# hongfz16/AvatarCLIP

Measured on AMD Instinct MI355X. Metric: rays_per_sec_512x512_64spp_clip_guided_train_iter, higher is better.
Workload: dtype f16 (forward) / bf16 (gradient sweeps) MFMA operands, fp32 accumulate

## Files before the change

### avatarclip_amd/build.py

```python
import os
import subprocess
import sys
from concurrent.futures import ThreadPoolExecutor

HERE = os.path.dirname(os.path.abspath(__file__))
CSRC = os.path.join(HERE, "csrc")
LIB = os.path.join(HERE, os.environ.get("AVC_LIB_NAME", "libavc.so"))
SOURCES = ["avc_core.hip", "avc_mlp_fwd.hip", "avc_mlp_bwd.hip", "avc_wgrad.hip", "avc_rays.hip", "avc_vit.hip", "avc_vit_attn.hip", "avc_vit_gemm.hip", "avc_mcubes.hip", "avc_raster.hip", "avc_raster_grad.hip", "avc_raster_tex.hip", "avc_params.hip", "avc_glue.hip", "avc_drive.hip", "avc_rig.hip", "avc_preview.hip", "avc_smpl.hip", "avc_smpl_grad.hip", "avc_codebook.hip", "avc_bake.hip", "avc_preview_clip.hip"]
ABI_HEADER = os.path.join("..", "..", "include", "avc.h")
TEXTURE_HEADER = "avc_texture.h"
CODEBOOK_HEADER = "avc_codebook.h"
PREVIEW_CLIP_HEADER = "avc_preview_clip.h"
BAKE_HEADER = "avc_bake.h"
HEADERS = ["avc_common.h", "avc_stage.h", "avc_mlp.h", "avc_bwd_body.h", "avc_offsets_gen.h", "avc_raster.h", "avc_raster_grad.h", "avc_smpl.h", "avc_vit.h", ABI_HEADER,
           TEXTURE_HEADER, CODEBOOK_HEADER, BAKE_HEADER, "avc_preview.h", PREVIEW_CLIP_HEADER]
FLAGS = ["--offload-arch=gfx950", "-O3", "-std=c++17", "-fPIC", "-Wno-comment"]


def _hipcc():
    for c in (os.environ.get("HIPCC"), "/opt/rocm/bin/hipcc", "hipcc"):
        if c and (os.path.isabs(c) and os.path.exists(c) or not os.path.isabs(c)):
            return c
    return "hipcc"


def _stale(target, deps):
    if not os.path.exists(target):
        return True
    t = os.path.getmtime(target)
    return any(os.path.getmtime(d) > t for d in deps if os.path.exists(d))


def _gen_offsets():
    import importlib.util
    spec = importlib.util.spec_from_file_location("gen_offsets", os.path.join(os.path.dirname(HERE), "scripts", "gen_offsets.py"))
    mod = importlib.util.module_from_spec(spec)
    spec.loader.exec_module(mod)
# ... 35 lines not shown
```

### avatarclip_amd/csrc/avc_wgrad.hip

```cpp
#include "avc_common.h"
#include "../../include/avc.h"
#include <type_traits>

#define WG_TB_MAX 9
#define WG_TILES_MAX 18
#define WG_BUF_BYTES (WG_TILES_MAX * 2048)
constexpr int WG_DEPTH = 4;
constexpr int WG_DMA_AUX = 2;

struct WgRegions { const char* base[2]; long stride[2]; };

typedef short vs4 __attribute__((__vector_size__(4 * sizeof(short))));
typedef __attribute__((address_space(3))) char lds_char;

__device__ __forceinline__ void wait_vmcnt(int n) {
#define WG_W(k) case k: asm volatile("s_waitcnt vmcnt(" #k ")" ::: "memory"); break;
  switch (n) {
    WG_W(0) WG_W(1) WG_W(2) WG_W(3) WG_W(4) WG_W(5) WG_W(6) WG_W(7) WG_W(8) WG_W(9) WG_W(10) WG_W(11) WG_W(12) WG_W(13) WG_W(14) WG_W(15)
    WG_W(16) WG_W(17) WG_W(18) WG_W(19) WG_W(20) WG_W(21) WG_W(22) WG_W(23) WG_W(24) WG_W(25) WG_W(26) WG_W(27) WG_W(28) WG_W(29) WG_W(30)
    WG_W(31) WG_W(32) WG_W(33) WG_W(34) WG_W(35) WG_W(36)
    default: asm volatile("s_waitcnt vmcnt(0)" ::: "memory"); break;
  }
#undef WG_W
}
// ... 111 lines not shown
    if (ta >= ta_n) continue;
#pragma unroll
    for (int k = 0; k < NK; ++k) {
      const int tb = wb + WB * k;
      if (tb >= tb_n) continue;
      f4* d4 = reinterpret_cast<f4*>(dst + ((long)(ta * tb_n + tb) * 64 + lane) * 16);
#pragma unroll
      for (int q = 0; q < 4; ++q) {
        f4 v;
        v[0] = acc[i * NK + k][4 * q]; v[1] = acc[i * NK + k][4 * q + 1]; v[2] = acc[i * NK + k][4 * q + 2]; v[3] = acc[i * NK + k][4 * q + 3];
        d4[q] = v;
      }
    }
    if (bias_partial && wb == i) {
      const float s = xhalf_sum(bsum[i]);
      if (lane < 32) bias_partial[(long)split * bias_elems + ta * 32 + lane] = s;
    }
  }
}

template <int N>
__device__ __forceinline__ void wait_vmcnt_imm() { asm volatile("s_waitcnt vmcnt(%0)" ::"n"(N) : "memory"); }

template <int MC, int TA, int TYA, int TYB>
struct WgCopies {
  const char* next[MC];
  long step[MC];
  unsigned src_lo;
  int wv;
  __device__ __forceinline__ WgCopies(const WgRegions& rg, int pa, int pb, long b0, int wv_, int lane) : wv(wv_) {
    src_lo = (((lane >> 2) & 3) * 32 + 4 * (lane >> 4) + (lane & 3)) * 16;
#pragma unroll
    for (int j = 0; j < MC; ++j) {
      const int c = wv + 8 * j, tix = c >> 1;
      const bool in_a = tix < TA;
      step[j] = in_a ? rg.stride[TYA] : rg.stride[TYB];
      next[j] = (in_a ? rg.base[TYA] + (long)(pa + tix) * 2048 : rg.base[TYB] + (long)(pb + tix - TA) * 2048) + b0 * step[j] + (c & 1) * 256;
    }
  }
  __device__ __forceinline__ void issue(char* lds, int slot) {
#pragma unroll
    for (int j = 0; j < MC; ++j) {
      asm("" : "+s"(next[j]));
      __builtin_amdgcn_global_load_lds((const __attribute__((address_space(1))) void*)(next[j] + src_lo),
                                       (__attribute__((address_space(3))) void*)(lds + slot * WG_BUF_BYTES + (wv + 8 * j) * 1024), 16, 0,
                                       WG_DMA_AUX);
      next[j] += step[j];
    }
  }
};

template <int MC, class Copies, class Contract>
__device__ __forceinline__ void wg_ring(char* lds, Copies& cp, long b0, long b1, Contract&& contract) {
  constexpr int depth = WG_DEPTH;
  const int n = (int)(b1 - b0);
  for (int d = 0; d < depth - 1; ++d)
    if (d < n) cp.issue(lds, d);
  int slot = 0;
  auto block = [&](auto ahead) {
    asm volatile("s_waitcnt lgkmcnt(0)" ::: "memory");
    __builtin_amdgcn_s_barrier();
    __builtin_amdgcn_sched_barrier(0);
    if constexpr (decltype(ahead)::value) cp.issue(lds, slot == 0 ? depth - 1 : slot - 1);
    contract(lds + slot * WG_BUF_BYTES);
    if (++slot == depth) slot = 0;
// ... 9 lines not shown
    wait_vmcnt(younger * MC);
    block(std::false_type{});
  }
}

__device__ __forceinline__ int wg_lane_off(int lane) {
  return (((lane >> 5) * 2) * 16 + (((lane >> 4) & 1) * 2 + (lane & 1)) * 4 + ((lane & 15) >> 2)) * 16 + 8 * ((lane & 3) >> 1);
}
__device__ __forceinline__ void wg_store_tile(float* dst, int tile, int lane, const facc& v16) {
  f4* d4 = reinterpret_cast<f4*>(dst + ((long)tile * 64 + lane) * 16);
#pragma unroll
  for (int q = 0; q < 4; ++q) {
    f4 v;
    v[0] = v16[4 * q]; v[1] = v16[4 * q + 1]; v[2] = v16[4 * q + 2]; v[3] = v16[4 * q + 3];
    d4[q] = v;
  }
}
__device__ __forceinline__ float wg_row_sum(float bsum, b8 s0, b8 s1) {
#pragma unroll
  for (int j = 0; j < 8; ++j) bsum += (float)s0[j] + (float)s1[j];
  return bsum;
}

template <int NI, int NK, int TA, int TB, int WA, int TYA, int TYB, bool BIAS, bool LASTA, bool LASTB, bool HI>
__device__ __forceinline__ void weight_grad_fixed(char* lds, const WgRegions& rg, int pa, int pb, long nblk, float* __restrict__ partial,
                                                  float* __restrict__ bias_partial, int out_elems, int bias_elems) {
  constexpr int WB = 8 / WA, nchunk = 2 * (TA + TB);
  constexpr int MC = HI ? (nchunk + 7) / 8 : nchunk / 8;
  constexpr int NIW = LASTA ? NI : NI - 1, NKW = LASTB ? NK : NK - 1;
  static_assert(WA * (NI - 1) < TA && WA * (NI - 2) + WA - 1 < TA && WB * (NK - 1) < TB && WB * (NK - 2) + WB - 1 < TB,
                "only the last slot of either side may be missing for some waves");
  const int lane = threadIdx.x & 63;
  const int wv = __builtin_amdgcn_readfirstlane((int)(threadIdx.x >> 6)) & 7;
  const int wa = wv % WA, wb = wv / WA;
  const int split = blockIdx.x, nsplit = gridDim.x;
  const long b0 = nblk * split / nsplit, b1 = nblk * (split + 1) / nsplit;
  WgCopies<MC, TA, TYA, TYB> cp(rg, pa, pb, b0, wv, lane);
  const int lane_off = wg_lane_off(lane);
  facc acc[NI * NK];
#pragma unroll
  for (int q = 0; q < NI * NK; ++q)
#pragma unroll
    for (int r = 0; r < 16; ++r) acc[q][r] = 0.f;
  float bsum = 0.f;
  wg_ring<MC>(lds, cp, b0, b1, [&](char* slot_buf) {
    lds_char* buf = (lds_char*)slot_buf + lane_off;
    b8 a[NI][2], bv[NK][2];
    auto read = [&](int t) {
#pragma unroll
      for (int i = 0; i < NIW; ++i) a[i][t] = tr_frag(buf + (wa + WA * i) * 2048, t);
#pragma unroll
      for (int k = 0; k < NKW; ++k) bv[k][t] = tr_frag(buf + (TA + wb + WB * k) * 2048, t);
    };
    auto convert = [&](int t) {
      if constexpr (TYA == 0) {
#pragma unroll
        for (int i = 0; i < NIW; ++i) a[i][t] = f16_to_bf16(a[i][t]);
      }
      if constexpr (TYB == 0) {
#pragma unroll
        for (int k = 0; k < NKW; ++k) bv[k][t] = f16_to_bf16(bv[k][t]);
      }
    };
    auto mfmas = [&](int t) {
#pragma unroll
      for (int i = 0; i < NIW; ++i)
#pragma unroll
        for (int k = 0; k < NKW; ++k) acc[i * NK + k] = MF<b8>::mma(a[i][t], bv[k][t], acc[i * NK + k]);
    };
    read(0);
    __builtin_amdgcn_sched_barrier(0);
    convert(0);
    __builtin_amdgcn_sched_barrier(0);
    read(1);
    mfmas(0);
    __builtin_amdgcn_sched_barrier(0);
    convert(1);
    mfmas(1);
    if constexpr (BIAS) {
      b8 s0 = a[0][0], s1 = a[0][1];
#pragma unroll
      for (int i = 1; i < NIW; ++i) { s0 = wb == i ? a[i][0] : s0; s1 = wb == i ? a[i][1] : s1; }
      bsum = wg_row_sum(bsum, s0, s1);
    }
  });
  float* dst = partial + (long)split * out_elems;
#pragma unroll
  for (int i = 0; i < NIW; ++i)
#pragma unroll
    for (int k = 0; k < NKW; ++k) wg_store_tile(dst, (wa + WA * i) * TB + wb + WB * k, lane, acc[i * NK + k]);
  if constexpr (BIAS) {
    if (wb < NIW) {
      const float s = xhalf_sum(bsum);
      if (lane < 32) bias_partial[(long)split * bias_elems + (wa + WA * wb) * 32 + lane] = s;
    }
  }
}

template <int NI, int NK, int TA, int TB, int WA, int TYA, int TYB, bool BIAS>
__device__ __forceinline__ void weight_grad_shipped(char* lds, const WgRegions& rg, int pa, int pb, long nblk, float* __restrict__ partial,
                                                    float* __restrict__ bias_partial, int out_elems, int bias_elems) {
  constexpr int WB = 8 / WA, nchunk = 2 * (TA + TB);
  constexpr bool role_a = WA * (NI - 1) + WA - 1 >= TA, role_b = WB * (NK - 1) + WB - 1 >= TB, role_hi = (nchunk & 7) != 0;
  const int wv = __builtin_amdgcn_readfirstlane((int)(threadIdx.x >> 6)) & 7;
  const bool lasta = !role_a || wv % WA + WA * (NI - 1) < TA, lastb = !role_b || wv / WA + WB * (NK - 1) < TB;
  const bool hi = !role_hi || wv < (nchunk & 7);
#define WG_ROLE(LA, LB, H)                                                                                                            \
  if ((LA || role_a) && (LB || role_b) && (H || role_hi) && lasta == LA && lastb == LB && hi == H)                                  \
    return weight_grad_fixed<NI, NK, TA, TB, WA, TYA, TYB, BIAS, LA || !role_a, LB || !role_b, H || !role_hi>(                        \
        lds, rg, pa, pb, nblk, partial, bias_partial, out_elems, bias_elems);
  WG_ROLE(true, true, true) WG_ROLE(true, true, false) WG_ROLE(true, false, true) WG_ROLE(true, false, false)
  WG_ROLE(false, true, true) WG_ROLE(false, true, false) WG_ROLE(false, false, true) WG_ROLE(false, false, false)
#undef WG_ROLE
}

template <int ROLE, int TYA, int TYB, bool BIAS>
__device__ __forceinline__ void weight_grad_fixed_9x9(char* lds, const WgRegions& rg, int pa, int pb, long nblk, float* __restrict__ partial,
                                                      float* __restrict__ bias_partial, int out_elems, int bias_elems) {
  constexpr int TA = 9, TB = 9;
  constexpr bool COL1 = ROLE >= 2, HAS_X = ROLE != 1;
  constexpr int MC = COL1 ? 4 : 5;
  constexpr int NR = COL1 ? 4 : 5;
  constexpr int XK = COL1 ? 0 : 4;
  const int lane = threadIdx.x & 63;
  const int wv = __builtin_amdgcn_readfirstlane((int)(threadIdx.x >> 6)) & 7;
  const int wa = wv & 3;
  const int split = blockIdx.x, nsplit = gridDim.x;
  const long b0 = nblk * split / nsplit, b1 = nblk * (split + 1) / nsplit;
  WgCopies<MC, TA, TYA, TYB> cp(rg, pa, pb, b0, wv, lane);
  const int lane_off = wg_lane_off(lane);
  int tb_of[NR];
#pragma unroll
  for (int k = 0; k < NR; ++k) tb_of[k] = COL1 ? 1 + 2 * ((wa + k) & 3) : 2 * k;
  facc acc[2 * NR], ex[2];
#pragma unroll
  for (int q = 0; q < 2 * NR; ++q)
// ... 198 lines not shown
      store_tile(wa, wb + 2 * k, acc[k]);
      store_tile(wa + 4, wb + 2 * k, acc[5 + k]);
    }
  }
  if (has_x) store_tile(8, wb + 2 * xk, ex[0]);
  if (wb == 1) store_tile(8, 2 * wa, ex[1]);
  if (bias_partial) {
#pragma unroll
    for (int i = 0; i < 2; ++i) {
      if (wb == i) {
        const float sx = xhalf_sum(bsum[i]);
        if (lane < 32) bias_partial[(long)split * bias_elems + (wa + 4 * i) * 32 + lane] = sx;
      }
    }
    if (wv == 4) {
      const float sx = xhalf_sum(xsum);
      if (lane < 32) bias_partial[(long)split * bias_elems + 8 * 32 + lane] = sx;
    }
  }
}

#define WG_MAX_PAIRS 24
struct WgPairs { int v[WG_MAX_PAIRS][8]; };
__global__ __launch_bounds__(512) void weight_grad_all_kernel(WgRegions rg, WgPairs pp, long nblk,
                                                              float* __restrict__ partial, float* __restrict__ bias_partial,
                                                              int out_elems, int bias_elems) {
  extern __shared__ __attribute__((aligned(16))) char lds[];
  const int* d = pp.v[blockIdx.y];
  float* bp = d[5] >= 0 ? bias_partial + d[5] : nullptr;
#define WG_ARGS lds, rg, d[0], d[1], d[2], d[3], d[6], d[7], nblk, partial + d[4], bp, out_elems, bias_elems
#define WG_SHIPPED(...) weight_grad_shipped<__VA_ARGS__>(lds, rg, d[0], d[2], nblk, partial + d[4], bp, out_elems, bias_elems)
  const bool gxf_bias = d[6] == 1 && d[7] == 0 && bp, fxg_plain = d[6] == 0 && d[7] == 1 && !bp;
  if (gxf_bias && d[1] == 8 && d[3] == 8) {
    WG_SHIPPED(4, 2, 8, 8, 2, 1, 0, true);
  } else if (fxg_plain && d[1] == 8 && d[3] == 8) {
    WG_SHIPPED(2, 4, 8, 8, 4, 0, 1, false);
  } else if (gxf_bias && d[1] == 7 && d[3] == 8) {
    WG_SHIPPED(4, 2, 7, 8, 2, 1, 0, true);
  } else if (fxg_plain && d[1] == 7 && d[3] == 8) {
    WG_SHIPPED(2, 4, 7, 8, 4, 0, 1, false);
  } else if (gxf_bias && d[1] == 8 && d[3] == 9) {
    WG_SHIPPED(2, 5, 8, 9, 4, 1, 0, true);
  } else if (gxf_bias && d[1] == 8 && d[3] == 2) {
    WG_SHIPPED(1, 2, 8, 2, 8, 1, 0, true);
  } else if (fxg_plain && d[1] == 8 && d[3] == 2) {
    WG_SHIPPED(1, 2, 8, 2, 8, 0, 1, false);
  } else if (gxf_bias && d[1] == 1 && d[3] == 8) {
    WG_SHIPPED(1, 1, 1, 8, 1, 1, 0, true);
  } else if (d[1] > 1 && d[3] > 2 && d[3] <= 8) {
    if (d[7] == 0) weight_grad_body<4, 2>(WG_ARGS, 2);
    else weight_grad_body<2, 4>(WG_ARGS, 4);
  } else if (gxf_bias && d[1] == 9 && d[3] == 9) {
    weight_grad_shipped_9x9<1, 0, true>(lds, rg, d[0], d[2], nblk, partial + d[4], bp, out_elems, bias_elems);
  } else if (d[1] == 9 && d[3] == 9) {
    weight_grad_body_9x9(lds, rg, d[0], d[2], d[6], d[7], nblk, partial + d[4], bp, out_elems, bias_elems);
  } else if (d[1] > 1 && d[3] > 8) {
    weight_grad_body<2, 5>(WG_ARGS, 4);
  } else if (d[1] > 1) {
    weight_grad_body<1, 2>(WG_ARGS, 8);
  } else {
    weight_grad_body<1, 2>(WG_ARGS, 1);
  }
#undef WG_SHIPPED
#undef WG_ARGS
}

extern "C" int avc_weight_grad_all(const void* fpanels, int ftiles, const void* gpanels, int gtiles, int npairs, const int* pairs,
                                   long nblk, float* partial, float* bias_partial, int nsplit, int out_stride, int bias_stride,
                                   void* stream) {
  if (nblk <= 0 || npairs <= 0) return 0;
  if (!fpanels || !gpanels) { avc_set_error("avc_weight_grad_all: fpanels / gpanels == NULL"); return 1; }
  if (npairs > WG_MAX_PAIRS) { avc_set_error("avc_weight_grad_all: too many pairs"); return 1; }
  WgPairs pp;
  for (int i = 0; i < npairs; ++i) {
    for (int k = 0; k < 8; ++k) pp.v[i][k] = pairs[i * 8 + k];
    const bool merged = pp.v[i][1] == 9 && pp.v[i][3] == 9;
    if (!merged && (pp.v[i][1] < 1 || pp.v[i][1] > 8 || pp.v[i][3] < 1 || pp.v[i][3] > WG_TB_MAX)) {
      avc_set_error("avc_weight_grad_all: 1 <= ta <= 8, 1 <= tb <= 9 (or the 9 x 9 product)");
      return 1;
    }
    const int* d = pp.v[i];
    if ((d[6] != 0 && d[6] != 1) || (d[7] != 0 && d[7] != 1)) {
      avc_set_error("avc_weight_grad_all: operand types are 0 (F region) or 1 (G region)");
      return 1;
    }
    const long tiles_a = d[6] ? gtiles : ftiles, tiles_b = d[7] ? gtiles : ftiles;
    if (d[0] < 0 || (long)d[0] + d[1] > tiles_a || d[2] < 0 || (long)d[2] + d[3] > tiles_b) {
      avc_set_error("avc_weight_grad_all: a pair's tiles lie outside their region");
      return 1;
    }
    if (d[4] < 0 || (long)d[4] + (long)d[1] * d[3] * 1024 > out_stride) {
      avc_set_error("avc_weight_grad_all: a pair's products lie outside out_stride");
      return 1;
    }
    if (d[5] >= 0 && (long)d[5] + 32 * d[1] > bias_stride) {
      avc_set_error("avc_weight_grad_all: a pair's bias sums lie outside bias_stride");
      return 1;
    }
  }
  if (nsplit < 1) nsplit = 1;
  const int lds_bytes = WG_DEPTH * WG_BUF_BYTES;
  static unsigned long long attr_seen = 0;
  if (avc_first_use_on_device(attr_seen)) {
    (void)hipFuncSetAttribute((const void*)weight_grad_all_kernel, hipFuncAttributeMaxDynamicSharedMemorySize, lds_bytes);
  }
  WgRegions rg;
  rg.base[0] = (const char*)fpanels; rg.stride[0] = (long)ftiles * 2048;
  rg.base[1] = (const char*)gpanels; rg.stride[1] = (long)gtiles * 2048;
  hipLaunchKernelGGL(weight_grad_all_kernel, dim3(nsplit, npairs), dim3(512), lds_bytes, (hipStream_t)stream, rg, pp, nblk, partial,
                     bias_partial, out_stride, bias_stride);
  return avc_check_launch("avc_weight_grad_all");
}

__global__ __launch_bounds__(256) void wgrad_reduce_kernel(const float* __restrict__ partial, const float* __restrict__ bpartial, int ns,
                                                           long stride, long bstride, int gout4, int gbias4, float* __restrict__ acc,
                                                           int accumulate) {
  const int j = blockIdx.x * 256 + threadIdx.x;
  if (j >= gout4 + gbias4) return;
  const f4* src = j < gout4 ? reinterpret_cast<const f4*>(partial) + j : reinterpret_cast<const f4*>(bpartial) + (j - gout4);
  const long st4 = (j < gout4 ? stride : bstride) >> 2;
  f4 a = {0.f, 0.f, 0.f, 0.f};
  int s = 0;
  for (; s + 8 <= ns; s += 8) {
    f4 v[8];
#pragma unroll
    for (int u = 0; u < 8; ++u) v[u] = __builtin_nontemporal_load(src + (long)(s + u) * st4);
#pragma unroll
    for (int u = 0; u < 8; ++u) a += v[u];
  }
  for (; s < ns; ++s) a += __builtin_nontemporal_load(src + (long)s * st4);
  f4* out = reinterpret_cast<f4*>(acc) + j;
  if (accumulate) a += *out;
  *out = a;
}
// ... 28 lines not shown
```

### avatarclip_amd/engine.py

```python
import ctypes
import os
import weakref

import numpy as np
import torch

from . import lib as L
from . import packing as PK


class _DevLayout:

    _cache = {}

    def __init__(self, lay: PK.Layout, device):
        t = lambda a, dt=None: torch.from_numpy(np.ascontiguousarray(a)).to(device)
        self.lay = lay
        self.idx16 = t(lay.idx16)
        self.scale16 = t(lay.scale16)
        self.idx32 = t(lay.idx32)
        self.scale32 = t(lay.scale32)
        self.un_src = t(lay.un_src)
        self.un_tgt = t(lay.un_tgt)
        self.un_scale = t(lay.un_scale)
# ... 145 lines not shown
        if device.type != "cuda":
            raise RuntimeError("avatarclip_amd runs its hot path on an MI355X; got device %s (no CPU fallback)" % device)
        self.spec = spec
        self.device = device
        self.lib = L.load()
        self.dl = _DevLayout.get(spec, device)
        self.net = spec.net_id
        assert self.lib.avc_num_offsets() == PK.OFF_COUNT
        self.fwd_tiles = self.lib.avc_fwd_panel_tiles(self.net)
        self.grad_tiles = self.lib.avc_grad_panel_tiles(self.net)
        assert (self.fwd_tiles, self.grad_tiles) == (self.dl.lay.panel["FTILES"], self.dl.lay.panel["GTILES"]), \
            "panel layout mismatch between packing.py and csrc/avc_mlp.h"
        assert self.lib.avc_bwd_colsum_floats(self.net) == self.dl.lay.cs_size, "column-sum layout mismatch between packing.py and csrc/avc_mlp.h"
        self._colsum = None
        self.mask_u16 = self.lib.avc_mask_u16_per_block(self.net)
        self.fwd_scr_bytes = self.lib.avc_fwd_scratch_bytes_per_wave(self.net)
        self._fwd_scratch = None
        self._fpanels = None
        self._gpanels = None
        self._partials = None
        self._bpartials = None
        self._masks = None
        self._pairs_host = PK.region_local_pairs(self.dl.lay)
        self._sdf_bias0 = int(self.dl.lay.pbase["sdf.b%d" % (spec.NMID + 2)])
        self._packed_key = None
        self._packed = None
        self._panel_owner = None
        self._last_pack = None
        self._colsum_scratch = None
        self._plan_key = None
        self._plan_val = None

    @classmethod
    def for_networks(cls, sdf_net, col_net):
        eng = cls._by_net.get(sdf_net)
        if eng is None:
            col_conf = col_net.conf if col_net is not None else dict(
                d_hidden=sdf_net.conf["d_hidden"], n_layers=int(sdf_net.conf["n_layers"]) - 2,
                mode="no_view_dir", multires_view=0)
            spec = PK.spec_from_conf(sdf_net.conf, col_conf)
            eng = cls(spec, next(sdf_net.parameters()).device)
            cls._by_net[sdf_net] = eng
        return eng

    class _Timed:
        def __init__(self, name, npts):
# ... 130 lines not shown
        weights = torch.empty(R, S, device=dev, dtype=f32)
        cdf = torch.empty(R, S, device=dev, dtype=f32)
        mid_z = torch.empty(R, S, device=dev, dtype=f32)
        inside = torch.empty(R, S, device=dev, dtype=f32)
        eik = torch.empty(R, 2, device=dev, dtype=f32)
        wstat = torch.empty(2, R, device=dev, dtype=f32)
        nsum = torch.empty(R, 3, device=dev, dtype=f32)
        L.call("avc_composite_fwd", sdf, nrm, rgb, z, rays_o, rays_d, R, S, inv_s, float(sample_dist), float(cos_anneal), bg, bg_mode, color, extra,
               weights, cdf, mid_z, inside, eik, wstat, nsum)
        return color, extra, weights, cdf, mid_z, inside, eik, wstat, nsum

    def composite_bwd(self, sdf, nrm, rgb, z, rays_o, rays_d, inv_s, sample_dist, cos_anneal, bg, bg_mode, d_color,
                      d_extra, d_w, d_n_up, eik_scale, d_wsum=None, d_nsum=None):
        R, S = z.shape
        dev, f32 = self.device, torch.float32
        d_sdf = torch.empty(R, S, device=dev, dtype=f32)
        d_n = torch.empty(R, S, 3, device=dev, dtype=f32)
        d_rgb = torch.empty(R, S, 6, device=dev, dtype=f32)
        d_inv = torch.empty(R, device=dev, dtype=f32)
        L.call("avc_composite_bwd", sdf, nrm, rgb, z, rays_o, rays_d, R, S, inv_s, float(sample_dist), float(cos_anneal), bg, bg_mode, d_color,
               d_extra, d_w, d_n_up, d_wsum, d_nsum, eik_scale, d_sdf, d_n, d_rgb, d_inv)
        return d_sdf, d_n, d_rgb, d_inv

    def slab_walk(self, pk: Packed, rays_o, rays_d, z, sample_dist, d_sdf, d_n, d_rgb, rgb, panels_valid=False):
        lay = self.dl.lay
        R, S = z.shape
        rays_per_chunk, rays_per_slab = self.plan(R, S)
        if rays_per_chunk < R:
            panels_valid = False
        self._panel_owner = None
        if self._partials is None:
            self._partials = torch.empty(256, lay.gout_size, device=self.device, dtype=torch.float32)
            self._bpartials = torch.empty(256, max(lay.gbias_size, 1), device=self.device, dtype=torch.float32)
        st = L.stream()
        esz = 4
        scratch_out = None
        cs_rows = int(self.lib.avc_bwd_colsum_rows(min(R, rays_per_slab) * S, self.MAX_BWD_WAVES))
        if self._colsum is None or self._colsum.shape[0] < cs_rows:
            self._colsum = torch.zeros(cs_rows, lay.cs_size, device=self.device, dtype=torch.float32)
        cs_total = None
        for c0 in range(0, R, rays_per_chunk):
            c1 = min(R, c0 + rays_per_chunk)
            if not panels_valid:
                if scratch_out is None:
                    scratch_out = (torch.empty(R, S, device=self.device), torch.empty(R, S, 3, device=self.device),
                                   torch.empty(R, S, 6, device=self.device))
                self.points_fwd_train(pk, rays_o, rays_d, z, sample_dist, c0, c1, out=scratch_out)
            fpanels, masks = self._bufs_f(((c1 - c0) * S + 31) // 32)
            for s0 in range(c0, c1, rays_per_slab):
                s1 = min(c1, s0 + rays_per_slab)
                npts = (s1 - s0) * S
                nblk = (npts + 31) // 32
                assert ((s0 - c0) * S) % 32 == 0, "slabs start on a 32-point block of their chunk"
                fblk0 = (s0 - c0) * S // 32
                fptr = fpanels.data_ptr() + fblk0 * self.fwd_tiles * 2048
                mptr = masks.data_ptr() + fblk0 * self.mask_u16 * 2
                gpanels = self._bufs_g(nblk)
                bwd_args = (self.net, None, rays_o.data_ptr() + s0 * 3 * esz, rays_d.data_ptr() + s0 * 3 * esz,
                            z.data_ptr() + s0 * z.stride(0) * esz, S, z.stride(0), float(sample_dist), npts, pk.w_bf16, pk.tab,
                            self.dl.offsets, d_sdf.data_ptr() + s0 * S * esz, d_n.data_ptr() + s0 * S * 3 * esz,
                            d_rgb.data_ptr() + s0 * S * 6 * esz, rgb.data_ptr() + s0 * S * 6 * esz, fptr, gpanels, mptr, self._colsum)
                rows = int(self.lib.avc_bwd_colsum_rows(npts, self.MAX_BWD_WAVES))
                with Engine._Timed("avc_render_points_bwd", npts):
                    L.call("avc_render_points_bwd", *bwd_args, self.MAX_BWD_WAVES, stream=st)
                cs_slab = self._colsum[:rows].sum(0)
                cs_total = cs_slab if cs_total is None else cs_total + cs_slab
                ns = max(1, min(self.WG_MAX_SPLITS, nblk // self.WG_BLOCKS_PER_SPLIT, nblk))
                with Engine._Timed("avc_weight_grad(all pairs)", npts):
                    L.call("avc_weight_grad_all", fptr, self.fwd_tiles, gpanels, self.grad_tiles, len(self._pairs_host), self._pairs_host.ctypes.data,
                           nblk, self._partials, self._bpartials, ns, self._partials.stride(0), self._bpartials.stride(0), stream=st)
                    yield ns, cs_total

    def points_bwd(self, pk: Packed, rays_o, rays_d, z, sample_dist, d_sdf, d_n, d_rgb, rgb, panels_valid=False):
        lay = self.dl.lay
        st = L.stream()
        gacc = torch.empty(lay.gout_size + lay.gbias_size, device=self.device, dtype=torch.float32)
        nslab, cs_total = 0, None
        for ns, cs_total in self.slab_walk(pk, rays_o, rays_d, z, sample_dist, d_sdf, d_n, d_rgb, rgb, panels_valid):
            L.call("avc_weight_grad_reduce", self._partials, self._bpartials, ns, self._partials.stride(0), self._bpartials.stride(0),
                   lay.gout_size, lay.gbias_size, gacc, int(nslab > 0), stream=st)
            nslab += 1
        grad = torch.empty(lay.nparam, device=self.device, dtype=torch.float32)
        if nslab == 0:
            grad.zero_()
        else:
            L.call("avc_weight_grad_unpack", gacc, self.dl.csr_off, self.dl.csr_src, self.dl.csr_scale, lay.nparam, grad, stream=st)
        if cs_total is not None:
            grad.index_add_(0, self.dl.cs_tgt, cs_total[self.dl.cs_src] * self.dl.cs_scale)
        if self.SDF_BIAS_FP32:
            grad[self._sdf_bias0] = d_sdf.sum()
        return grad


def eikonal_from_sums(sums, group):
    import torch.distributed as dist
    dist.all_reduce(sums, op=dist.ReduceOp.SUM, group=group)
    den = sums[1] + 1e-5
    return sums[0] / den, den


class RenderCoreFn(torch.autograd.Function):
# ... 58 lines not shown
```

### avatarclip_amd/lib.py

```python
import collections
import ctypes
import os
import re

import torch

from . import build as _build

_lib = None
_launches = {}
ABI_VERSION = None
HEADER = os.path.normpath(os.path.join(_build.CSRC, _build.ABI_HEADER))
TEXTURE_HEADER = os.path.join(_build.CSRC, _build.TEXTURE_HEADER)
CODEBOOK_HEADER = os.path.join(_build.CSRC, _build.CODEBOOK_HEADER)


PREVIEW_CLIP_HEADER = os.path.join(_build.CSRC, _build.PREVIEW_CLIP_HEADER)
BAKE_HEADER = os.path.join(_build.CSRC, _build.BAKE_HEADER)


def headers():
    return (HEADER, TEXTURE_HEADER, CODEBOOK_HEADER)


def added_headers():
    return (PREVIEW_CLIP_HEADER,)


def later_headers():
    return (BAKE_HEADER,)


c_int, c_long, c_float, c_double, c_void_p, c_char_p = (ctypes.c_int, ctypes.c_long, ctypes.c_float, ctypes.c_double,
                                                        ctypes.c_void_p, ctypes.c_char_p)

_SCALARS = {"int": c_int, "long": c_long, "float": c_float, "double": c_double}
_RETURNS = {"int": c_int, "long": c_long, "const char*": c_char_p}
_INTS = [getattr(torch, n) for n in ("bool", "int8", "uint8", "int16", "uint16", "int32", "uint32", "int64", "uint64") if hasattr(torch, n)]
_FLOAT32, _FLOAT64 = frozenset([torch.float32]), frozenset([torch.float64])
_INT1, _INT4, _INT8 = (frozenset(d for d in _INTS if d.itemsize == n) for n in (1, 4, 8))
_ELEMENTS = {"float": _FLOAT32, "double": _FLOAT64, "int": _INT4, "unsigned": _INT4, "long": _INT8, "long long": _INT8, "unsigned long long": _INT8,
             "void*": _INT8, "signed char": _INT1, "unsigned char": _INT1, "void": None}
_TYPE_WORDS = {"const", "void", "char", "short", "int", "long", "float", "double", "signed", "unsigned"}

Param = collections.namedtuple("Param", "name ctype decl elem const")


class Proto(collections.namedtuple("Proto", "name restype params")):
    @property
    def argtypes(self):
        return [p.ctype for p in self.params]

    @property
# ... 72 lines not shown
            env["_ok%d" % i] = _ELEMENTS[q.elem]
            exprs.append(_POINTER.format(a=a, i=i, dtype="" if _ELEMENTS[q.elem] is None else "%s.dtype in _ok%d and " % (a, i)))
        else:
            exprs.append(a)
    exprs.append("_current_stream().cuda_stream if stream is None else stream")
    exec("def %s(%s*, stream=None):\n    if _fn(%s) != 0:\n        _failed()\n"
         % (proto.name, "".join(n + ", " for n in names), ",\n           ".join(exprs)), env)
    return env[proto.name]


def lib_path():
    return _build.LIB


def load():
    global _lib, ABI_VERSION
    if _lib is not None:
        return _lib
    path = lib_path()
    if not os.path.exists(path):
        raise RuntimeError("libavc.so is not built (run `python -c 'import __graft_entry__ as g; g.build()'`); "
                           "there is no CPU fallback for the HIP hot path")
    protos, declared_in = {}, {}
    for header in headers() + added_headers() + later_headers():
        with open(header) as f:
            more, abi = parse_header(f.read())
        if header == HEADER:
            ABI_VERSION = abi
        twice = sorted(set(more) & set(protos))
        if twice:
            raise RuntimeError("%s declares %s, which %s declares already" % (header, ", ".join(twice), declared_in[twice[0]]))
        protos.update(more)
        declared_in.update((name, header) for name in more)
    lib = ctypes.CDLL(path)
    got = lib.avc_version()
    if got != ABI_VERSION:
        raise RuntimeError("%s implements revision %d of include/avc.h, this binding expects %s: rebuild the library "
                           "(python -m avatarclip_amd.build --force)" % (path, got, ABI_VERSION))
    for name, proto in protos.items():
        fn = getattr(lib, name, None)
        if fn is None:
            where = ("include/" if declared_in[name] == HEADER else "csrc/") + os.path.basename(declared_in[name])
            raise RuntimeError("%s implements revision %d of include/avc.h but lacks %s of %s: rebuild the library "
                               "(python -m avatarclip_amd.build --force)" % (path, got, name, where))
        fn.restype = proto.restype
        fn.argtypes = proto.argtypes
    _launches.update((name, bind(proto, getattr(lib, name))) for name, proto in protos.items() if proto.launch)
# ... 29 lines not shown
```

### avatarclip_amd/packing.py

```python
import math
import os
import re
from dataclasses import dataclass, field
from functools import lru_cache
from typing import Dict, List, Tuple

import numpy as np

SQ2 = math.sqrt(2.0)
S_B2 = 100.0 * math.log2(math.e)
_HERE = os.path.dirname(os.path.abspath(__file__))


def _parse_offsets_enum() -> Dict[str, int]:
    src = open(os.path.join(_HERE, "csrc", "avc_common.h")).read()
    body = re.search(r"enum AvcOff \{(.*?)\};", src, re.S).group(1)
    body = re.sub(r"//[^\n]*", "", body)
    names = [n.strip().split("=")[0].strip() for n in body.split(",") if n.strip()]
    return {n: i for i, n in enumerate(names)}


OFF = _parse_offsets_enum()
OFF_COUNT = OFF["OFF_COUNT"]

# ... 144 lines not shown
class Layout:
    spec: NetSpec
    shapes: List[Tuple[str, Tuple[int, ...]]]
    pbase: Dict[str, int]
    nparam: int
    idx16: np.ndarray
    scale16: np.ndarray
    idx32: np.ndarray
    scale32: np.ndarray
    offsets: np.ndarray
    panel: Dict[str, int]
    pairs: List[Tuple[int, int, int, int, int, int, int, int]]
    gout_size: int
    gbias_size: int
    un_src: np.ndarray
    un_tgt: np.ndarray
    un_scale: np.ndarray
    ub_src: np.ndarray
    ub_tgt: np.ndarray
    cs_size: int = 0
    cs_src: np.ndarray = None
    cs_tgt: np.ndarray = None
    cs_scale: np.ndarray = None


def _elem(pbase, name, shape, row, col, transposed):
    ld = shape[1]
    return pbase[name] + (col * ld + row if transposed else row * ld + col)


@lru_cache(maxsize=None)
def build_layout(H: int, NMID: int, NCMID: int) -> Layout:
    spec = NetSpec(H, NMID, NCMID)
    shapes = param_shapes(spec)
    pbase, n = {}, 0
    for name, shp in shapes:
        pbase[name] = n
        n += int(np.prod(shp))
    ZERO = n
    shp = dict(shapes)
    HT, HK, SKIP, ST, SK = spec.HT, spec.HK, spec.SKIP, spec.ST, spec.SK
    ls, ll = "sdf.W%d" % (NMID + 1), "sdf.W%d" % (NMID + 2)
    bs, bl = "sdf.b%d" % (NMID + 1), "sdf.b%d" % (NMID + 2)

    idx16, sc16, offsets = [], [], np.zeros(OFF_COUNT, np.int32)
    cur16 = [0]
# ... 204 lines not shown
        return lambda f: a(f) if f < 32 * ST else b(f - 32 * ST)
    hs_scale = lambda t_b: 1 / (SQ2 * S_B2) if t_b < ST else 1 / SQ2
    assert P["SDF"] == P["DFEAT"] + HT
    rows_last = lambda f: r1(f) if f < 32 * HT else r0s(f - 32 * HT)
    add_pair(P["DFEAT"], HT + 1, P["HS"], ST + 2, ll, rows_last, last_cols(True), scale=hs_scale, bname=bl)
    cs_src, cs_tgt = [], []
    for t in range(ST):
        for h in range(2):
            for r in range(16):
                f = 32 * t + acc_row(r, h)
                if f < SKIP:
                    cs_src.append((t * 2 + h) * 16 + r)
                    cs_tgt.append(pbase[ll] + f)
    for q in range(24):
        for h in range(2):
            f = pe_feat(h, q, False)
            if f >= 0:
                cs_src.append(ST * 32 + ((q >> 3) * 2 + h) * 8 + (q & 7))
                cs_tgt.append(pbase[ll] + SKIP + f)
    assert len(set(cs_tgt)) == len(cs_tgt) == SKIP + 39, "every column of row 0 exactly once"
    fx = feat_xn()
    c0col = lambda f: (6 + f) if f < H else fx(f - H)
    add_pair(P["D1"], HT, P["FEAT"], HT + 1, "col.W0", feat_std(H), c0col, bname="col.b0")
    if NCMID == 1:
        add_pair(P["D2"], HT, P["R1"], HT, "col.W1", feat_std(H), feat_std(H), bname="col.b1")
        add_pair(P["DO"], 1, P["R2"], HT, "col.Wh", feat_std(6), feat_std(H), bname="col.bh")
    else:
        add_pair(P["DO"], 1, P["R1"], HT, "col.Wh", feat_std(6), feat_std(H), bname="col.bh")

    return Layout(spec=spec, shapes=shapes, pbase=pbase, nparam=n,
                  idx16=np.concatenate(idx16), scale16=np.concatenate(sc16),
                  idx32=np.concatenate(idx32), scale32=np.concatenate(sc32), offsets=offsets, panel=P, pairs=pairs,
                  gout_size=gout[0], gbias_size=gbias[0],
                  un_src=np.concatenate(un_src), un_tgt=np.concatenate(un_tgt), un_scale=np.concatenate(un_scale),
                  ub_src=np.asarray(ub_src, np.int64), ub_tgt=np.asarray(ub_tgt, np.int64),
                  cs_size=ST * 32 + 48, cs_src=np.asarray(cs_src, np.int64), cs_tgt=np.asarray(cs_tgt, np.int64),
                  cs_scale=np.full(len(cs_src), 1 / SQ2, np.float32))


def layout_for(spec: NetSpec) -> Layout:
    return build_layout(spec.H, spec.NMID, spec.NCMID)


def region_local_pairs(lay: Layout) -> np.ndarray:
    ft = lay.panel["FTILES"]
    out = np.asarray(lay.pairs, dtype=np.int32).reshape(-1, 8).copy()
    out[:, 0] -= np.where(out[:, 6] == 1, ft, 0)
    out[:, 2] -= np.where(out[:, 7] == 1, ft, 0)
    assert (out[:, 0] >= 0).all() and (out[:, 2] >= 0).all()
    return np.ascontiguousarray(out)
```

Baseline: 2.461 million.

## Rebuild the D2 gradient panel inside the weight-grad kernel from delta_o and masks

For the col.W1 weight-gradient pair (8x8 tiles, bias), the kernel no longer streams the precomputed D2 gradient A-tiles from global memory. It loads the head-weight tile once, streams the delta_o tile and ReLU mask words, recomputes D2 = W_h^T·delta_o with an MFMA, applies the mask, and writes the bf16 result straight into the LDS ring slot next to the DMA'd F tiles. This cuts global reads of the D2 panel for that pair at the cost of an extra MFMA, mask handling and a more intricate pipelined schedule. The host gains a new ABI entry and uses it by default when the layout qualifies.

```diff
diff --git a/avatarclip_amd/build.py b/avatarclip_amd/build.py
--- a/avatarclip_amd/build.py
+++ b/avatarclip_amd/build.py
@@ -12,7 +12,8 @@
 CODEBOOK_HEADER = "avc_codebook.h"
 PREVIEW_CLIP_HEADER = "avc_preview_clip.h"
 BAKE_HEADER = "avc_bake.h"
-HEADERS = ["avc_common.h", "avc_stage.h", "avc_mlp.h", "avc_bwd_body.h", "avc_offsets_gen.h", "avc_raster.h", "avc_raster_grad.h", "avc_smpl.h", "avc_vit.h", ABI_HEADER,
+WGRAD_HEADER = "avc_wgrad.h"
+HEADERS = ["avc_common.h", "avc_stage.h", "avc_mlp.h", "avc_bwd_body.h", "avc_offsets_gen.h", "avc_raster.h", "avc_raster_grad.h", "avc_smpl.h", "avc_vit.h", WGRAD_HEADER, ABI_HEADER,
            TEXTURE_HEADER, CODEBOOK_HEADER, BAKE_HEADER, "avc_preview.h", PREVIEW_CLIP_HEADER]
 FLAGS = ["--offload-arch=gfx950", "-O3", "-std=c++17", "-fPIC", "-Wno-comment"]
 
diff --git a/avatarclip_amd/csrc/avc_wgrad.h b/avatarclip_amd/csrc/avc_wgrad.h
--- /dev/null
+++ b/avatarclip_amd/csrc/avc_wgrad.h
@@ -0,0 +1,15 @@
+#ifndef AVC_WGRAD_H
+#define AVC_WGRAD_H
+#ifdef __cplusplus
+extern "C" {
+#endif
+
+int avc_weight_grad_all_rebuilt(const void* fpanels, int ftiles, const void* gpanels, int gtiles, int npairs,
+                                const int* pairs , long nblk, float* partial, float* bias_partial, int nsplit,
+                                int out_stride, int bias_stride, int rebuilt_pair, int do_tile, const void* head_tiles,
+                                const void* masks, int mask_stride, int mask_first, void* stream);
+
+#ifdef __cplusplus
+}
+#endif
+#endif
diff --git a/avatarclip_amd/csrc/avc_wgrad.hip b/avatarclip_amd/csrc/avc_wgrad.hip
--- a/avatarclip_amd/csrc/avc_wgrad.hip
+++ b/avatarclip_amd/csrc/avc_wgrad.hip
@@ -1,5 +1,6 @@
 #include "avc_common.h"
 #include "../../include/avc.h"
+#include "avc_wgrad.h"
 #include <type_traits>
 
 #define WG_TB_MAX 9
@@ -157,7 +158,7 @@
 template <int N>
 __device__ __forceinline__ void wait_vmcnt_imm() { asm volatile("s_waitcnt vmcnt(%0)" ::"n"(N) : "memory"); }
 
-template <int MC, int TA, int TYA, int TYB>
+template <int MC, int TA, int TYA, int TYB, int J0 = 0>
 struct WgCopies {
   const char* next[MC];
   long step[MC];
@@ -166,7 +167,7 @@
   __device__ __forceinline__ WgCopies(const WgRegions& rg, int pa, int pb, long b0, int wv_, int lane) : wv(wv_) {
     src_lo = (((lane >> 2) & 3) * 32 + 4 * (lane >> 4) + (lane & 3)) * 16;
 #pragma unroll
-    for (int j = 0; j < MC; ++j) {
+    for (int j = J0; j < MC; ++j) {
       const int c = wv + 8 * j, tix = c >> 1;
       const bool in_a = tix < TA;
       step[j] = in_a ? rg.stride[TYA] : rg.stride[TYB];
@@ -175,7 +176,7 @@
   }
   __device__ __forceinline__ void issue(char* lds, int slot) {
 #pragma unroll
-    for (int j = 0; j < MC; ++j) {
+    for (int j = J0; j < MC; ++j) {
       asm("" : "+s"(next[j]));
       __builtin_amdgcn_global_load_lds((const __attribute__((address_space(1))) void*)(next[j] + src_lo),
                                        (__attribute__((address_space(3))) void*)(lds + slot * WG_BUF_BYTES + (wv + 8 * j) * 1024), 16, 0,
@@ -231,6 +232,49 @@
   return bsum;
 }
 
+template <int NI, int NK, int NIW, int NKW, int TA, int WA, int TYA, int TYB, bool BIAS>
+struct WgBlock {
+  static constexpr int WB = 8 / WA;
+  lds_char* buf;
+  int wa, wb;
+  b8 a[NI][2], bv[NK][2];
+  __device__ __forceinline__ void read(int t) {
+#pragma unroll
+    for (int i = 0; i < NIW; ++i) a[i][t] = tr_frag(buf + (wa + WA * i) * 2048, t);
+#pragma unroll
+    for (int k = 0; k < NKW; ++k) bv[k][t] = tr_frag(buf + (TA + wb + WB * k) * 2048, t);
+  }
+  __device__ __forceinline__ void convert(int t) {
+    if constexpr (TYA == 0) {
+#pragma unroll
+      for (int i = 0; i < NIW; ++i) a[i][t] = f16_to_bf16(a[i][t]);
+    }
+    if constexpr (TYB == 0) {
+#pragma unroll
+      for (int k = 0; k < NKW; ++k) bv[k][t] = f16_to_bf16(bv[k][t]);
+    }
+  }
+  __device__ __forceinline__ void mfmas(int t, facc (&acc)[NI * NK]) {
+#pragma unroll
+    for (int i = 0; i < NIW; ++i)
+#pragma unroll
+      for (int k = 0; k < NKW; ++k) acc[i * NK + k] = MF<b8>::mma(a[i][t], bv[k][t], acc[i * NK + k]);
+  }
+  __device__ __forceinline__ void rest(facc (&acc)[NI * NK], float& bsum) {
+    read(1);
+    mfmas(0, acc);
+    __builtin_amdgcn_sched_barrier(0);
+    convert(1);
+    mfmas(1, acc);
+    if constexpr (BIAS) {
+      b8 s0 = a[0][0], s1 = a[0][1];
+#pragma unroll
+      for (int i = 1; i < NIW; ++i) { s0 = wb == i ? a[i][0] : s0; s1 = wb == i ? a[i][1] : s1; }
+      bsum = wg_row_sum(bsum, s0, s1);
+    }
+  }
+};
+
 template <int NI, int NK, int TA, int TB, int WA, int TYA, int TYB, bool BIAS, bool LASTA, bool LASTB, bool HI>
 __device__ __forceinline__ void weight_grad_fixed(char* lds, const WgRegions& rg, int pa, int pb, long nblk, float* __restrict__ partial,
                                                   float* __restrict__ bias_partial, int out_elems, int bias_elems) {
@@ -253,45 +297,12 @@
     for (int r = 0; r < 16; ++r) acc[q][r] = 0.f;
   float bsum = 0.f;
   wg_ring<MC>(lds, cp, b0, b1, [&](char* slot_buf) {
-    lds_char* buf = (lds_char*)slot_buf + lane_off;
-    b8 a[NI][2], bv[NK][2];
-    auto read = [&](int t) {
-#pragma unroll
-      for (int i = 0; i < NIW; ++i) a[i][t] = tr_frag(buf + (wa + WA * i) * 2048, t);
-#pragma unroll
-      for (int k = 0; k < NKW; ++k) bv[k][t] = tr_frag(buf + (TA + wb + WB * k) * 2048, t);
-    };
-    auto convert = [&](int t) {
-      if constexpr (TYA == 0) {
-#pragma unroll
-        for (int i = 0; i < NIW; ++i) a[i][t] = f16_to_bf16(a[i][t]);
-      }
-      if constexpr (TYB == 0) {
-#pragma unroll
-        for (int k = 0; k < NKW; ++k) bv[k][t] = f16_to_bf16(bv[k][t]);
-      }
-    };
-    auto mfmas = [&](int t) {
-#pragma unroll
-      for (int i = 0; i < NIW; ++i)
-#pragma unroll
-        for (int k = 0; k < NKW; ++k) acc[i * NK + k] = MF<b8>::mma(a[i][t], bv[k][t], acc[i * NK + k]);
-    };
-    read(0);
+    WgBlock<NI, NK, NIW, NKW, TA, WA, TYA, TYB, BIAS> blk{(lds_char*)slot_buf + lane_off, wa, wb};
+    blk.read(0);
     __builtin_amdgcn_sched_barrier(0);
-    convert(0);
+    blk.convert(0);
     __builtin_amdgcn_sched_barrier(0);
-    read(1);
-    mfmas(0);
-    __builtin_amdgcn_sched_barrier(0);
-    convert(1);
-    mfmas(1);
-    if constexpr (BIAS) {
-      b8 s0 = a[0][0], s1 = a[0][1];
-#pragma unroll
-      for (int i = 1; i < NIW; ++i) { s0 = wb == i ? a[i][0] : s0; s1 = wb == i ? a[i][1] : s1; }
-      bsum = wg_row_sum(bsum, s0, s1);
-    }
+    blk.rest(acc, bsum);
   });
   float* dst = partial + (long)split * out_elems;
 #pragma unroll
@@ -321,6 +332,129 @@
   WG_ROLE(true, true, true) WG_ROLE(true, true, false) WG_ROLE(true, false, true) WG_ROLE(true, false, false)
   WG_ROLE(false, true, true) WG_ROLE(false, true, false) WG_ROLE(false, false, true) WG_ROLE(false, false, false)
 #undef WG_ROLE
+}
+
+struct WgRebuild {
+  const b8* wht;
+  const unsigned short* masks;
+  long mask_stride;
+  int pair;
+  int g_do;
+};
+typedef unsigned wg_u4 __attribute__((ext_vector_type(4)));
+
+__device__ __forceinline__ void weight_grad_rebuilt(char* lds, const WgRegions& rg, const WgRebuild& rb, int pb, long nblk,
+                                                    float* __restrict__ partial, float* __restrict__ bias_partial, int out_elems,
+                                                    int bias_elems) {
+  constexpr int NI = 4, NK = 2, TA = 8, TB = 8, WA = 2;
+  constexpr int MC = 2 * (TA + TB) / 8, J0 = 2 * TA / 8;
+  constexpr int VM = MC - J0 + 2;
+  const int lane = threadIdx.x & 63;
+  const int wv = __builtin_amdgcn_readfirstlane((int)(threadIdx.x >> 6)) & 7;
+  const int wa = wv % WA, wb = wv / WA;
+  const int split = blockIdx.x, nsplit = gridDim.x;
+  const long b0 = nblk * split / nsplit, b1 = nblk * (split + 1) / nsplit;
+  const int n = (int)(b1 - b0);
+  WgCopies<MC, TA, 1, 0, J0> cp(rg, 0, pb, b0, wv, lane);
+  const int lane_off = wg_lane_off(lane);
+  const unsigned wr_off = (unsigned)(wv * 2048 + ((((lane & 31) >> 2) * 16 + (lane >> 5) * 4 + (lane & 3)) * 16));
+  b8 aw = as_global(rb.wht)[wv * 64 + lane];
+  asm volatile("" : "+v"(aw));
+  const char* dof_next = rg.base[1] + (long)rb.g_do * 2048 + b0 * rg.stride[1];
+  const unsigned short* mk_next = rb.masks + b0 * rb.mask_stride + wv * 64;
+  b8 dofr[3];
+  unsigned mkr[3] = {0u, 0u, 0u};
+#pragma unroll
+  for (int s = 0; s < 3; ++s)
+#pragma unroll
+    for (int j = 0; j < 8; ++j) dofr[s][j] = (__bf16)0.f;
+  facc acc[NI * NK];
+#pragma unroll
+  for (int q = 0; q < NI * NK; ++q)
+#pragma unroll
+    for (int r = 0; r < 16; ++r) acc[q][r] = 0.f;
+  float bsum = 0.f;
+  const unsigned dof_off = (unsigned)lane * 16u, mk_off = (unsigned)lane * 2u;
+  auto load = [&](auto set, auto steady) {
+    constexpr int s = decltype(set)::value;
+    asm("" : "+s"(dof_next), "+s"(mk_next));
+    if constexpr (decltype(steady)::value) {
+      asm volatile("global_load_dwordx4 %0, %2, %3\n\tglobal_load_ushort %1, %4, %5"
+                   : "+v"(dofr[s]), "+v"(mkr[s]) : "v"(dof_off), "s"(dof_next), "v"(mk_off), "s"(mk_next) : "memory");
+    } else {
+      dofr[s] = *reinterpret_cast<const AVC_GLOBAL b8*>(as_global(dof_next) + dof_off);
+      mkr[s] = *reinterpret_cast<const AVC_GLOBAL unsigned short*>(as_global(reinterpret_cast<const char*>(mk_next)) + mk_off);
+    }
+    dof_next += rg.stride[1];
+    mk_next += rb.mask_stride;
+  };
+  auto product = [&](auto set) {
+    facc z;
+#pragma unroll
+    for (int r = 0; r < 16; ++r) z[r] = 0.f;
+    return MF<b8>::mma(aw, dofr[decltype(set)::value], z);
+  };
+  auto store = [&](auto set, const facc& d, int slot) {
+    const unsigned bits = mkr[decltype(set)::value];
+    b8 f0, f1;
+#pragma unroll
+    for (int j = 0; j < 8; ++j) {
+      f0[j] = (__bf16)(((bits >> relu_mask_bit(j)) & 1u) ? d[j] : 0.f);
+      f1[j] = (__bf16)(((bits >> relu_mask_bit(8 + j)) & 1u) ? d[8 + j] : 0.f);
+    }
+    const unsigned at = (unsigned)(uintptr_t)(lds_char*)lds + (unsigned)slot * WG_BUF_BYTES + wr_off;
+    asm volatile("ds_write_b128 %0, %1\n\tds_write_b128 %0, %2 offset:128"
+                 :: "v"(at), "v"(__builtin_bit_cast(wg_u4, f0)), "v"(__builtin_bit_cast(wg_u4, f1)) : "memory");
+  };
+  typedef std::integral_constant<int, 0> S0;
+  typedef std::integral_constant<int, 1> S1;
+  typedef std::integral_constant<int, 2> S2;
+  if (0 < n) { load(S0{}, std::false_type{}); cp.issue(lds, 0); }
+  if (1 < n) { load(S1{}, std::false_type{}); cp.issue(lds, 1); }
+  if (2 < n) { load(S2{}, std::false_type{}); cp.issue(lds, 2); }
+  store(S0{}, product(S0{}), 0);
+  int k = 0, slot = 0;
+  auto block = [&](auto set, auto steady) {
+    typedef std::integral_constant<int, (decltype(set)::value + 1) % 3> Use;
+    if constexpr (decltype(steady)::value) {
+      wait_vmcnt_imm<(WG_DEPTH - 2) * VM - 2>();
+    } else {
+      const int younger = n - 1 - k;
+      if (younger >= 2) wait_vmcnt_imm<(WG_DEPTH - 2) * VM - 2>();
+      else if (younger == 1) wait_vmcnt_imm<MC - J0>();
+      else wait_vmcnt_imm<0>();
+    }
+    asm volatile("s_waitcnt lgkmcnt(0)" ::: "memory");
+    __builtin_amdgcn_s_barrier();
+    __builtin_amdgcn_sched_barrier(0);
+    asm volatile("" : "+v"(dofr[Use::value]), "+v"(mkr[Use::value]));
+    if (decltype(steady)::value || k + WG_DEPTH - 1 < n) { load(set, steady); cp.issue(lds, slot == 0 ? WG_DEPTH - 1 : slot - 1); }
+    const facc d = product(Use{});
+    WgBlock<NI, NK, NI, NK, TA, WA, 1, 0, true> blk{(lds_char*)(lds + slot * WG_BUF_BYTES) + lane_off, wa, wb};
+    blk.read(0);
+    __builtin_amdgcn_sched_barrier(0);
+    store(Use{}, d, slot == WG_DEPTH - 1 ? 0 : slot + 1);
+    blk.convert(0);
+    __builtin_amdgcn_sched_barrier(0);
+    blk.rest(acc, bsum);
+    ++k;
+    if (++slot == WG_DEPTH) slot = 0;
+  };
+  for (; k + WG_DEPTH + 1 < n;) { block(S0{}, std::true_type{}); block(S1{}, std::true_type{}); block(S2{}, std::true_type{}); }
+  for (; k < n;) {
+    block(S0{}, std::false_type{});
+    if (k < n) block(S1{}, std::false_type{});
+    if (k < n) block(S2{}, std::false_type{});
+  }
+  float* dst = partial + (long)split * out_elems;
+#pragma unroll
+  for (int i = 0; i < NI; ++i)
+#pragma unroll
+    for (int q = 0; q < NK; ++q) wg_store_tile(dst, (wa + WA * i) * TB + wb + (8 / WA) * q, lane, acc[i * NK + q]);
+  if (wb < NI) {
+    const float s = xhalf_sum(bsum);
+    if (lane < 32) bias_partial[(long)split * bias_elems + (wa + WA * wb) * 32 + lane] = s;
+  }
 }
 
 template <int ROLE, int TYA, int TYB, bool BIAS>
@@ -565,7 +699,7 @@
 
 #define WG_MAX_PAIRS 24
 struct WgPairs { int v[WG_MAX_PAIRS][8]; };
-__global__ __launch_bounds__(512) void weight_grad_all_kernel(WgRegions rg, WgPairs pp, long nblk,
+__global__ __launch_bounds__(512) void weight_grad_all_kernel(WgRegions rg, WgPairs pp, WgRebuild rb, long nblk,
                                                               float* __restrict__ partial, float* __restrict__ bias_partial,
                                                               int out_elems, int bias_elems) {
   extern __shared__ __attribute__((aligned(16))) char lds[];
@@ -575,7 +709,8 @@
 #define WG_SHIPPED(...) weight_grad_shipped<__VA_ARGS__>(lds, rg, d[0], d[2], nblk, partial + d[4], bp, out_elems, bias_elems)
   const bool gxf_bias = d[6] == 1 && d[7] == 0 && bp, fxg_plain = d[6] == 0 && d[7] == 1 && !bp;
   if (gxf_bias && d[1] == 8 && d[3] == 8) {
-    WG_SHIPPED(4, 2, 8, 8, 2, 1, 0, true);
+    if ((int)blockIdx.y == rb.pair) weight_grad_rebuilt(lds, rg, rb, d[2], nblk, partial + d[4], bp, out_elems, bias_elems);
+    else WG_SHIPPED(4, 2, 8, 8, 2, 1, 0, true);
   } else if (fxg_plain && d[1] == 8 && d[3] == 8) {
     WG_SHIPPED(2, 4, 8, 8, 4, 0, 1, false);
   } else if (gxf_bias && d[1] == 7 && d[3] == 8) {
@@ -608,9 +743,9 @@
 #undef WG_ARGS
 }
 
-extern "C" int avc_weight_grad_all(const void* fpanels, int ftiles, const void* gpanels, int gtiles, int npairs, const int* pairs,
-                                   long nblk, float* partial, float* bias_partial, int nsplit, int out_stride, int bias_stride,
-                                   void* stream) {
+static int weight_grad_launch(const void* fpanels, int ftiles, const void* gpanels, int gtiles, int npairs, const int* pairs, long nblk,
+                              float* partial, float* bias_partial, int nsplit, int out_stride, int bias_stride, const WgRebuild& rb,
+                              void* stream) {
   if (nblk <= 0 || npairs <= 0) return 0;
   if (!fpanels || !gpanels) { avc_set_error("avc_weight_grad_all: fpanels / gpanels == NULL"); return 1; }
   if (npairs > WG_MAX_PAIRS) { avc_set_error("avc_weight_grad_all: too many pairs"); return 1; }
@@ -650,9 +785,42 @@
   WgRegions rg;
   rg.base[0] = (const char*)fpanels; rg.stride[0] = (long)ftiles * 2048;
   rg.base[1] = (const char*)gpanels; rg.stride[1] = (long)gtiles * 2048;
-  hipLaunchKernelGGL(weight_grad_all_kernel, dim3(nsplit, npairs), dim3(512), lds_bytes, (hipStream_t)stream, rg, pp, nblk, partial,
+  if (rb.pair >= 0) {
+    const int* d = rb.pair < npairs ? pp.v[rb.pair] : nullptr;
+    if (!d || d[1] != 8 || d[3] != 8 || d[6] != 1 || d[7] != 0 || d[5] < 0) {
+      avc_set_error("avc_weight_grad_all_rebuilt: rebuilt_pair must name an 8 x 8 product of G-region A tiles and F-region B tiles with bias");
+      return 1;
+    }
+    if (!rb.wht || !rb.masks) { avc_set_error("avc_weight_grad_all_rebuilt: head_tiles / masks == NULL"); return 1; }
+    if (rb.g_do < 0 || rb.g_do >= gtiles) { avc_set_error("avc_weight_grad_all_rebuilt: the delta_o tile lies outside the G region"); return 1; }
+  }
+  hipLaunchKernelGGL(weight_grad_all_kernel, dim3(nsplit, npairs), dim3(512), lds_bytes, (hipStream_t)stream, rg, pp, rb, nblk, partial,
                      bias_partial, out_stride, bias_stride);
   return avc_check_launch("avc_weight_grad_all");
+}
+extern "C" int avc_weight_grad_all(const void* fpanels, int ftiles, const void* gpanels, int gtiles, int npairs, const int* pairs,
+                                   long nblk, float* partial, float* bias_partial, int nsplit, int out_stride, int bias_stride,
+                                   void* stream) {
+  WgRebuild rb = {nullptr, nullptr, 0, -1, 0};
+  return weight_grad_launch(fpanels, ftiles, gpanels, gtiles, npairs, pairs, nblk, partial, bias_partial, nsplit, out_stride, bias_stride,
+                            rb, stream);
+}
+extern "C" int avc_weight_grad_all_rebuilt(const void* fpanels, int ftiles, const void* gpanels, int gtiles, int npairs, const int* pairs,
+                                           long nblk, float* partial, float* bias_partial, int nsplit, int out_stride, int bias_stride,
+                                           int rebuilt_pair, int do_tile, const void* head_tiles, const void* masks, int mask_stride,
+                                           int mask_first, void* stream) {
+  if (rebuilt_pair < 0) { avc_set_error("avc_weight_grad_all_rebuilt: rebuilt_pair < 0 (avc_weight_grad_all launches without one)"); return 1; }
+  if (((uintptr_t)head_tiles & 15) || ((uintptr_t)masks & 1)) {
+    avc_set_error("avc_weight_grad_all_rebuilt: head_tiles must be 16-byte aligned, masks 2-byte aligned");
+    return 1;
+  }
+  if (mask_first < 0 || mask_stride < 0 || (long)mask_first + 8 * 64 > mask_stride) {
+    avc_set_error("avc_weight_grad_all_rebuilt: the 8 x 64 mask words of a block lie outside mask_stride");
+    return 1;
+  }
+  WgRebuild rb = {(const b8*)head_tiles, masks ? (const unsigned short*)masks + mask_first : nullptr, (long)mask_stride, rebuilt_pair, do_tile};
+  return weight_grad_launch(fpanels, ftiles, gpanels, gtiles, npairs, pairs, nblk, partial, bias_partial, nsplit, out_stride, bias_stride,
+                            rb, stream);
 }
 
 __global__ __launch_bounds__(256) void wgrad_reduce_kernel(const float* __restrict__ partial, const float* __restrict__ bpartial, int ns,
diff --git a/avatarclip_amd/engine.py b/avatarclip_amd/engine.py
--- a/avatarclip_amd/engine.py
+++ b/avatarclip_amd/engine.py
@@ -191,6 +191,7 @@
         self._bpartials = None
         self._masks = None
         self._pairs_host = PK.region_local_pairs(self.dl.lay)
+        self._rebuilt = PK.rebuilt_pair_args(self.dl.lay)
         self._sdf_bias0 = int(self.dl.lay.pbase["sdf.b%d" % (spec.NMID + 2)])
         self._packed_key = None
         self._packed = None
@@ -367,7 +368,17 @@
                d_extra, d_w, d_n_up, d_wsum, d_nsum, eik_scale, d_sdf, d_n, d_rgb, d_inv)
         return d_sdf, d_n, d_rgb, d_inv
 
-    def slab_walk(self, pk: Packed, rays_o, rays_d, z, sample_dist, d_sdf, d_n, d_rgb, rgb, panels_valid=False):
+    def weight_grad_all(self, pk: Packed, fptr, gpanels, mptr, nblk, ns, rebuild=True, stream=None):
+        head = (fptr, self.fwd_tiles, gpanels, self.grad_tiles, len(self._pairs_host), self._pairs_host.ctypes.data, nblk, self._partials,
+                self._bpartials, ns, self._partials.stride(0), self._bpartials.stride(0))
+        if rebuild and self._rebuilt is not None:
+            pair, do_tile, w_off, mask_first = self._rebuilt
+            L.call("avc_weight_grad_all_rebuilt", *head, pair, do_tile, pk.w_bf16.data_ptr() + w_off, mptr, self.mask_u16, mask_first,
+                   stream=stream)
+        else:
+            L.call("avc_weight_grad_all", *head, stream=stream)
+
+    def slab_walk(self, pk: Packed, rays_o, rays_d, z, sample_dist, d_sdf, d_n, d_rgb, rgb, panels_valid=False, rebuild=True):
         lay = self.dl.lay
         R, S = z.shape
         rays_per_chunk, rays_per_slab = self.plan(R, S)
@@ -412,16 +423,15 @@
                 cs_total = cs_slab if cs_total is None else cs_total + cs_slab
                 ns = max(1, min(self.WG_MAX_SPLITS, nblk // self.WG_BLOCKS_PER_SPLIT, nblk))
                 with Engine._Timed("avc_weight_grad(all pairs)", npts):
-                    L.call("avc_weight_grad_all", fptr, self.fwd_tiles, gpanels, self.grad_tiles, len(self._pairs_host), self._pairs_host.ctypes.data,
-                           nblk, self._partials, self._bpartials, ns, self._partials.stride(0), self._bpartials.stride(0), stream=st)
+                    self.weight_grad_all(pk, fptr, gpanels, mptr, nblk, ns, rebuild, stream=st)
                     yield ns, cs_total
 
-    def points_bwd(self, pk: Packed, rays_o, rays_d, z, sample_dist, d_sdf, d_n, d_rgb, rgb, panels_valid=False):
+    def points_bwd(self, pk: Packed, rays_o, rays_d, z, sample_dist, d_sdf, d_n, d_rgb, rgb, panels_valid=False, rebuild=True):
         lay = self.dl.lay
         st = L.stream()
         gacc = torch.empty(lay.gout_size + lay.gbias_size, device=self.device, dtype=torch.float32)
         nslab, cs_total = 0, None
-        for ns, cs_total in self.slab_walk(pk, rays_o, rays_d, z, sample_dist, d_sdf, d_n, d_rgb, rgb, panels_valid):
+        for ns, cs_total in self.slab_walk(pk, rays_o, rays_d, z, sample_dist, d_sdf, d_n, d_rgb, rgb, panels_valid, rebuild):
             L.call("avc_weight_grad_reduce", self._partials, self._bpartials, ns, self._partials.stride(0), self._bpartials.stride(0),
                    lay.gout_size, lay.gbias_size, gacc, int(nslab > 0), stream=st)
             nslab += 1
diff --git a/avatarclip_amd/lib.py b/avatarclip_amd/lib.py
--- a/avatarclip_amd/lib.py
+++ b/avatarclip_amd/lib.py
@@ -17,6 +17,7 @@
 
 PREVIEW_CLIP_HEADER = os.path.join(_build.CSRC, _build.PREVIEW_CLIP_HEADER)
 BAKE_HEADER = os.path.join(_build.CSRC, _build.BAKE_HEADER)
+WGRAD_HEADER = os.path.join(_build.CSRC, _build.WGRAD_HEADER)
 
 
 def headers():
@@ -29,6 +30,10 @@
 
 def later_headers():
     return (BAKE_HEADER,)
+
+
+def wgrad_headers():
+    return (WGRAD_HEADER,)
 
 
 c_int, c_long, c_float, c_double, c_void_p, c_char_p = (ctypes.c_int, ctypes.c_long, ctypes.c_float, ctypes.c_double,
@@ -147,7 +152,7 @@
         raise RuntimeError("libavc.so is not built (run `python -c 'import __graft_entry__ as g; g.build()'`); "
                            "there is no CPU fallback for the HIP hot path")
     protos, declared_in = {}, {}
-    for header in headers() + added_headers() + later_headers():
+    for header in headers() + added_headers() + later_headers() + wgrad_headers():
         with open(header) as f:
             more, abi = parse_header(f.read())
         if header == HEADER:
diff --git a/avatarclip_amd/packing.py b/avatarclip_amd/packing.py
--- a/avatarclip_amd/packing.py
+++ b/avatarclip_amd/packing.py
@@ -190,6 +190,7 @@
     cs_src: np.ndarray = None
     cs_tgt: np.ndarray = None
     cs_scale: np.ndarray = None
+    rebuilt: dict = None
 
 
 def _elem(pbase, name, shape, row, col, transposed):
@@ -440,8 +441,11 @@
     fx = feat_xn()
     c0col = lambda f: (6 + f) if f < H else fx(f - H)
     add_pair(P["D1"], HT, P["FEAT"], HT + 1, "col.W0", feat_std(H), c0col, bname="col.b0")
+    rebuilt = None
     if NCMID == 1:
         add_pair(P["D2"], HT, P["R1"], HT, "col.W1", feat_std(H), feat_std(H), bname="col.b1")
+        if HT == 8:
+            rebuilt = dict(pair=len(pairs) - 1, do_tile=P["DO"], weight_off="OFF_CHT", mask_layer=1, mask_first=1 * HT * 64)
         add_pair(P["DO"], 1, P["R2"], HT, "col.Wh", feat_std(6), feat_std(H), bname="col.bh")
     else:
         add_pair(P["DO"], 1, P["R1"], HT, "col.Wh", feat_std(6), feat_std(H), bname="col.bh")
@@ -453,7 +457,7 @@
                   un_src=np.concatenate(un_src), un_tgt=np.concatenate(un_tgt), un_scale=np.concatenate(un_scale),
                   ub_src=np.asarray(ub_src, np.int64), ub_tgt=np.asarray(ub_tgt, np.int64),
                   cs_size=ST * 32 + 48, cs_src=np.asarray(cs_src, np.int64), cs_tgt=np.asarray(cs_tgt, np.int64),
-                  cs_scale=np.full(len(cs_src), 1 / SQ2, np.float32))
+                  cs_scale=np.full(len(cs_src), 1 / SQ2, np.float32), rebuilt=rebuilt)
 
 
 def layout_for(spec: NetSpec) -> Layout:
@@ -467,3 +471,14 @@
     out[:, 2] -= np.where(out[:, 7] == 1, ft, 0)
     assert (out[:, 0] >= 0).all() and (out[:, 2] >= 0).all()
     return np.ascontiguousarray(out)
+
+
+def rebuilt_pair_args(lay: Layout):
+    rb = lay.rebuilt
+    if rb is None:
+        return None
+    pa, ta, _, tb, _, bias_off, type_a, type_b = lay.pairs[rb["pair"]]
+    assert (pa, ta, tb, type_a, type_b) == (lay.panel["D2"], 8, 8, 1, 0) and bias_off >= 0 and lay.spec.NCMID == 1
+    off = int(lay.offsets[OFF[rb["weight_off"]]])
+    assert off % 8 == 0, "a packed tile starts on a 16-byte fragment"
+    return rb["pair"], rb["do_tile"] - lay.panel["FTILES"], off * 2, rb["mask_first"]
```

Measured after the change: 2.466 million (median of 3 runs). No clear change (+0.2%).
